# MDFahimAnjum/AliasFree-Diffusion-Models-PyTorch

Measured on AMD Instinct MI355X. Metric: train_step_images_per_sec, higher is better.
Workload: dtype f32; 1 GPU; CIFAR-10 32x32x3 synthetic, UNet variant=3 (Config D), batch 256/GPU, T=1000, AdamW lr 3e-4, random-init weights (seed 42); global_batch=256, parallelism=dp1, hip_graph=True, launch_mode=lanes

## Files before the change

### aliasfree-diffusion-models-pytorch_amd/csrc/conv.hip

```cpp
#include <cstdlib>
#include <algorithm>
#include "common.h"

namespace afd {

using f32x16 = __attribute__((ext_vector_type(16))) float;

static inline int gs_grid(long total, int block = 256) {
  long g = (total + block - 1) / block;
  return (int)(g < 1 ? 1 : (g > 65536 ? 65536 : g));
}

template <int KS>
__global__ void conv_direct_fwd(const float* __restrict__ x, const float* __restrict__ w, const float* __restrict__ bias,
                                const float* __restrict__ res, float* __restrict__ y,
                                int Cin, int Cout, int H, int W, int act, long total) {
  constexpr int T = KS * KS, R = KS / 2;
  for (long i = blockIdx.x * (long)blockDim.x + threadIdx.x; i < total; i += (long)gridDim.x * blockDim.x) {
    const int xx = i % W, yy = (i / W) % H;
    const long bc = i / ((long)W * H);
    const int co = bc % Cout; const long b = bc / Cout;
    float acc = bias ? bias[co] : 0.f;
    for (int ci = 0; ci < Cin; ++ci) {
      const float* xp = x + (b * Cin + ci) * (long)H * W;
// ... 695 lines not shown
  if (nb > 0) d[nd++] = afd_fold_desc{bp, db, (long)nb, (long)nb, (long)nb, 1L, slabs, accumulate};
  if (sink) {
    for (int i = 0; i < nd; ++i) sink->out[sink->n++] = d[i];
    return AFD_OK;
  }
  return fold_launch(d, nd, s);
}

bool pw_launch(const float* in, const float* w, const float* bias, const float* res, float* out, int B, int K, int N, int P,
               int act, bool dgrad, hipStream_t s);
void pw_set_mode(int m);
int wino_plan(int B, int K, int N, int H, int W);
int wino_conv(const float* x, const float* w, const float* bias, const float* res, float* y, float* U, int B, int K, int N, int H,
               int W, int act, bool dgrad, bool weights_ready, hipStream_t s);
void wino_set_mode(int m);
void wino_weights_launch(const float* w, float* Uf, float* Ud, int Cin, int Cout, int kinds, hipStream_t s);
bool bf3_ok(int B, int K, int N, int H, int W);
void bf3_set_mode(int m);
void direct_form_set(int m);
bool direct_form_is_bf3();
void h2_sk_set_mode(int m);
void h2_lds_set(int m);
void h2_skw_set(int m);
void wino_weights_batched_launch(const afd_wino_desc* descs, const int* wg_desc, int n_wg, hipStream_t s);
void wino_set_grid(int g);
int wgrad_wino_plan(int B, int Cin, int Cout, int H, int W, int* bn, int* bk, int* cps, int* nchunks);
int wgrad_bf3_plan(int B, int Cin, int Cout, int H, int W, int* tps, int* ntiles);
int wgrad_bf3(const float* x, const float* dy, float* part, int B, int Cin, int Cout, int H, int W, hipStream_t s);
void wgrad_bf3_set_mode(int m);
void wgrad_arith_set(int m);
void wgrad_plan_target_set(long wgs);
bool wgrad_arith_is_bf3();
int wgrad_h2(const float* x, const float* dy, float* part, int B, int Cin, int Cout, int H, int W, hipStream_t s);
int pw_wgrad_h2(const float* x, const float* dy, float* part, float* bias_part, int B, int Cin, int Cout, int L, hipStream_t s);
bool ends_fwd(const float* x, const float* w, const float* bias, const float* res, float* y, int B, int Cin, int Cout, int H, int W,
              int ksize, int act, hipStream_t s);
bool ends_dgrad(const float* dy, const float* w, float* dx, int B, int Cin, int Cout, int H, int W, int ksize, hipStream_t s);
void ends_set_mode(int m);
int wgrad_cin3_plan(int B, int Cin, int Cout, int H, int W);
int wgrad_cin3(const float* x, const float* dy, float* part, int B, int Cin, int Cout, int H, int W, hipStream_t s);
void pw_wgrad_bf3_set_mode(int m);
int pw_wgrad_bf3_plan(int B, int Cin, int Cout, int L, int* sps, int* nsteps, int* nr, int* nt);
int pw_wgrad_bf3(const float* x, const float* dy, float* part, float* bias_part, int B, int Cin, int Cout, int L, hipStream_t s);
int wgrad_wino(const float* x, const float* dy, float* part, int B, int Cin, int Cout, int H, int W, hipStream_t s);
void wgrad_wino_set_mode(int m);

static inline bool use_mfma(int K, int N, int H, int W, int PT) { return N >= 8 && tile_ok(H, W, PT); }

static int g_conv_path = 0;

template <int T, bool DGRAD>
static int launch_mfma(const float* x, const float* w, const float* bias, const float* res, float* y,
                       int B, int K, int N, int H, int W, int act, hipStream_t s) {
  constexpr int KC = (T == 9) ? 8 : 32;
  const long P = (long)B * H * W;
  if (P * K >= (1L << 31) || (long)K * N * T >= (1L << 31)) return -1;
  const unsigned ptiles = (unsigned)((P + 127) / 128);
  const long wgs64 = (long)ptiles * ((N + 63) / 64), wgs32 = (long)ptiles * ((N + 31) / 32);
  bool use32 = N <= 32 || (wgs64 < 256 && wgs32 >= 256);
  const bool want_sk = g_conv_path == 2 || (g_conv_path == 0 && wgs64 < 256 && wgs32 < 256);
  if (g_conv_path == 1) use32 = N <= 32;
  if (want_sk && K >= 32 && tile_ok(H, W, 64)) {
    const TileGeom g = make_geom(H, W, 64, T == 9 ? 1 : 0);
    if (g.XS <= 256) {
      const size_t lds_main = sizeof(float) * (32 * (32 * T + 1) + (size_t)32 * g.XS);
      const size_t lds_red = sizeof(float) * 4 * 2 * 16 * 64;
// ... 50 lines not shown

template <int T, int WNn, int WCn, int NPB>
static void launch_wgrad(const float* x, const float* dy, float* part, float* bias_part, int B, int Cin, int Cout, int H, int W,
                         const WgradPlan& p, const TileGeom& g, hipStream_t s) {
  const int nw = g_wgrad_nw ? g_wgrad_nw : ((p.cps >= 8 || (p.cps >= 4 && H * W >= 256)) ? 8 : 4);
  size_t lds = sizeof(float) * ((size_t)32 * WNn * 65 + (size_t)32 * WCn * (g.XS | 1)) + sizeof(int) * 64;
  const size_t red = sizeof(float) * nw * 16 * 64;
  if (WNn * WCn < nw && lds < red) lds = red;
  const dim3 grid((Cout + 32 * WNn - 1) / (32 * WNn), (Cin + 32 * WCn - 1) / (32 * WCn), p.splits);
  if (nw == 8)
    hipLaunchKernelGGL((conv_wgrad_mfma<T, WNn, WCn, NPB, 8>), grid, dim3(512), lds, s, x, dy, part, bias_part, B, Cin, Cout, H, W, p.cps, p.nchunks, g);
  else
    hipLaunchKernelGGL((conv_wgrad_mfma<T, WNn, WCn, NPB, 4>), grid, dim3(256), lds, s, x, dy, part, bias_part, B, Cin, Cout, H, W, p.cps, p.nchunks, g);
}

template <int T, int NPB>
static void launch_wgrad_roles(const float* x, const float* dy, float* part, float* bp, int B, int Cin, int Cout, int H, int W,
                               const WgradPlan& p, const TileGeom& g, hipStream_t s) {
  if (p.wnn == 2 && p.wcn == 2) launch_wgrad<T, 2, 2, NPB>(x, dy, part, bp, B, Cin, Cout, H, W, p, g, s);
  else if (p.wnn == 2) launch_wgrad<T, 2, 1, NPB>(x, dy, part, bp, B, Cin, Cout, H, W, p, g, s);
  else if (p.wcn == 2) launch_wgrad<T, 1, 2, NPB>(x, dy, part, bp, B, Cin, Cout, H, W, p, g, s);
  else launch_wgrad<T, 1, 1, NPB>(x, dy, part, bp, B, Cin, Cout, H, W, p, g, s);
}

}
using namespace afd;

extern "C" {

int afd_debug_conv_path(int mode) {
  if (mode >= 92 && mode <= 93) { ends_set_mode(mode - 92); return AFD_OK; }
  if (mode >= 88 && mode <= 89) { pw_wgrad_bf3_set_mode(mode - 88); return AFD_OK; }
  if (mode >= 84 && mode <= 86) { wgrad_bf3_set_mode(mode - 84); return AFD_OK; }
  if (mode >= 48 && mode <= 49) { wgrad_plan_target_set(mode == 48 ? 256 : 160); return AFD_OK; }
  if (mode >= 59 && mode <= 63) { h2_lds_set(mode == 59 ? 4 : (mode == 60 ? 1 : (mode == 61 ? 0 : mode - 60))); return AFD_OK; }
  if (mode == 73) { h2_sk_set_mode(2); return AFD_OK; }
  if (mode >= 71 && mode <= 72) { h2_skw_set(mode - 70); return AFD_OK; }
  if (mode == 74) h2_skw_set(0);
  if (mode >= 74 && mode <= 75) { h2_sk_set_mode(mode - 74); return AFD_OK; }
  if (mode >= 78 && mode <= 79) { wgrad_arith_set(mode - 78); return AFD_OK; }
  if (mode >= 76 && mode <= 77) { direct_form_set(mode - 76); return AFD_OK; }
  if (mode >= 80 && mode <= 82) { bf3_set_mode(mode - 80); return AFD_OK; }
  if (mode >= 8 && mode <= 10) { pw_set_mode(mode - 8); return AFD_OK; }
  if (mode >= 100000 && mode < 200000) { wino_set_grid(mode - 100000); return AFD_OK; }
  if (mode >= 96 && mode <= 98) { wgrad_wino_set_mode(mode - 96); return AFD_OK; }
  if (mode >= 64 && mode <= 70) { wino_set_mode(mode - 64); return AFD_OK; }
  if (mode >= 32 && mode <= 34) { g_wgrad_nw = mode == 32 ? 4 : (mode == 33 ? 8 : 0); return AFD_OK; }
  AFD_REQUIRE(mode >= 0 && mode <= 2, "afd_debug_conv_path: mode must be 0 (auto), 1 (big tile), 2 (split-K tile), 8..10 (1x1 streaming auto/off/forced), 32..34 (wgrad waves 4/8/auto), 64..69 (Winograd fwd/dgrad auto/off/forced shapes) or 96..98 (Winograd wgrad auto/off/forced)");
  g_conv_path = mode;
  return AFD_OK;
}

int afd_conv_fwd(const float* x, const float* w, const float* bias, const float* res, float* y,
                 int B, int Cin, int Cout, int H, int W, int ksize, int act, afd_stream_t st) {
  AFD_REQUIRE(x && w && y && B > 0 && Cin > 0 && Cout > 0 && H > 0 && W > 0, "afd_conv_fwd: bad argument");
  AFD_REQUIRE(ksize == 1 || ksize == 3, "afd_conv_fwd: ksize %d not in {1,3}", ksize);
  AFD_REQUIRE(act == 0 || act == 1, "afd_conv_fwd: act must be 0 or 1");
  hipStream_t s = as_stream(st);
  if (ends_fwd(x, w, bias, res, y, B, Cin, Cout, H, W, ksize, act, s)) return check_launch("afd_conv_fwd");
  if (ksize == 1 && pw_launch(x, w, bias, res, y, B, Cin, Cout, H * W, act, false, s)) return check_launch("afd_conv_fwd");
  int rc = -1;
  if (use_mfma(Cin, Cout, H, W, 128))
    rc = ksize == 3 ? launch_mfma<9, false>(x, w, bias, res, y, B, Cin, Cout, H, W, act, s)
                    : launch_mfma<1, false>(x, w, bias, res, y, B, Cin, Cout, H, W, act, s);
  if (rc != 0) {
    const long total = (long)B * Cout * H * W;
// ... 92 lines not shown
    const size_t ws = (size_t)wgrad_wino_plan(B, Cin, Cout, H, W, &bn, &bk, &cps, &nch);
    if (ws > slabs) slabs = ws;
    const size_t wb = (size_t)wgrad_bf3_plan(B, Cin, Cout, H, W, &cps, &nch);
    if (wb > slabs) slabs = wb;
    const size_t wc = (size_t)wgrad_cin3_plan(B, Cin, Cout, H, W);
    if (wc > slabs) slabs = wc;
  }
  const size_t need = slabs * ((size_t)Cout * Cin * ksize * ksize + Cout);
  const size_t direct = (size_t)B * Cout;
  return std::max(pw, sizeof(float) * (need > direct ? need : direct));
}

int afd_conv_wgrad_form(int B, int Cin, int Cout, int H, int W, int ksize) {
  if (B <= 0 || Cin <= 0 || Cout <= 0 || H <= 0 || W <= 0) return 0;
  int a, b, c, d;
  if (ksize == 1) return pw_wgrad_bf3_plan(B, Cin, Cout, H * W, &a, &b, &c, &d) ? (wgrad_arith_is_bf3() ? 2 : 4) : 0;
  if (ksize != 3) return 0;
  if (wgrad_bf3_plan(B, Cin, Cout, H, W, &a, &b)) return wgrad_arith_is_bf3() ? 2 : 4;
  if (wgrad_cin3_plan(B, Cin, Cout, H, W)) return 3;
  return wgrad_wino_plan(B, Cin, Cout, H, W, &a, &b, &c, &d) ? 1 : 0;
}

static int conv_wgrad_impl(const float* x, const float* dy, float* dw, float* dbias, int B, int Cin, int Cout, int H, int W,
                           int ksize, int accumulate, void* workspace, FoldSink* sink, hipStream_t s, const char* who) {
  AFD_REQUIRE(x && dy && dw && B > 0 && Cin > 0 && Cout > 0 && H > 0 && W > 0, "%s: bad argument", who);
  AFD_REQUIRE(ksize == 1 || ksize == 3, "%s: ksize %d not in {1,3}", who, ksize);
  const int T = ksize * ksize;
  const TileGeom g = make_geom(H, W, 64, ksize == 3 ? 1 : 0);
  int rc = AFD_OK;
  const bool vec = aligned16(x) && aligned16(dy);
  if (ksize == 3 && !dbias && workspace) {
    float* part = static_cast<float*>(workspace);
    int slabs = !vec ? 0 : (wgrad_arith_is_bf3() ? wgrad_bf3(x, dy, part, B, Cin, Cout, H, W, s) : wgrad_h2(x, dy, part, B, Cin, Cout, H, W, s));
    if (!slabs) slabs = wgrad_cin3(x, dy, part, B, Cin, Cout, H, W, s);
    if (!slabs && vec) slabs = wgrad_wino(x, dy, part, B, Cin, Cout, H, W, s);
    if (slabs) {
      const long n = (long)Cout * Cin * 9;
      rc = launch_wgrad_reduce(part, dw, n, slabs, nullptr, nullptr, 0, accumulate, 9, s, sink);
      return rc != AFD_OK ? rc : check_launch(who);
    }
  }
  if (ksize == 1 && workspace && vec) {
    int a, b, c, d;
    const int slabs = pw_wgrad_bf3_plan(B, Cin, Cout, H * W, &a, &b, &c, &d);
    if (slabs) {
      float* part = static_cast<float*>(workspace);
      const long n = (long)Cout * Cin;
      float* bp = dbias ? part + (size_t)slabs * n : nullptr;
      if (wgrad_arith_is_bf3()) pw_wgrad_bf3(x, dy, part, bp, B, Cin, Cout, H * W, s);
      else pw_wgrad_h2(x, dy, part, bp, B, Cin, Cout, H * W, s);
      rc = launch_wgrad_reduce(part, dw, n, slabs, bp, dbias, dbias ? Cout : 0, accumulate, 1, s, sink);
      return rc != AFD_OK ? rc : check_launch(who);
    }
  }
  if (tile_ok(H, W, 64) && g.XS <= 256 && (long)B * H * W * (Cin > Cout ? Cin : Cout) < (1L << 31)) {
    AFD_REQUIRE(workspace, "%s: workspace is NULL", who);
    const WgradPlan p = wgrad_plan(B, Cin, Cout, H, W, ksize);
    float* part = static_cast<float*>(workspace);
    const long n = (long)Cout * Cin * T;
    float* bp = dbias ? part + (size_t)p.slabs * n : nullptr;
    if (ksize == 1) launch_wgrad_roles<1, 2>(x, dy, part, bp, B, Cin, Cout, H, W, p, g, s);
    else if (p.npb == 4) launch_wgrad_roles<9, 4>(x, dy, part, bp, B, Cin, Cout, H, W, p, g, s);
    else if (p.npb == 5) launch_wgrad_roles<9, 5>(x, dy, part, bp, B, Cin, Cout, H, W, p, g, s);
    else launch_wgrad_roles<9, 8>(x, dy, part, bp, B, Cin, Cout, H, W, p, g, s);
    rc = launch_wgrad_reduce(part, dw, n, p.slabs, bp, dbias, dbias ? Cout : 0, accumulate, T, s, sink);
    return rc != AFD_OK ? rc : check_launch(who);
// ... 31 lines not shown
```

### aliasfree-diffusion-models-pytorch_amd/csrc/h2_wgrad.hip

```cpp
#include <algorithm>
#include <cstdint>
#include <cstdlib>
#include "common.h"
#include "h2_common.h"

namespace afd {

using f32x4 = __attribute__((ext_vector_type(4))) float;
using u32x4 = __attribute__((ext_vector_type(4))) uint32_t;

template <int S, int BN_, int BK_> struct HwGeo {
  static constexpr int TP = 128, G8 = S / 8;
  static constexpr int IPT = S * S >= TP ? 1 : TP / (S * S);
  static constexpr int R = S * S >= TP ? TP / S : S;
  static constexpr int TPI = S * S >= TP ? S * S / TP : 1;
  static constexpr int IG = (R + 2) * G8, NG = IPT * IG;
  static constexpr int BK = BK_, BN = BN_;
  static constexpr int NR = (BN / 16) * (BK / 32), NSG = 8 / NR;
  static constexpr int TASKS = (BK / 16) * NG * 16, NE = (TASKS + 511) / 512;
  static constexpr int PIECE = (BK / 16) * NG * 16;
};

__device__ __forceinline__ uint32_t h_pack(_Float16 lo, _Float16 hi) {
  return (uint32_t)__builtin_bit_cast(uint16_t, lo) | ((uint32_t)__builtin_bit_cast(uint16_t, hi) << 16);
}

template <int NR, int NSG>
__device__ __forceinline__ void hw_finish(f32x4 (&acc)[2][9], float unscale_x, float unscale_d, uint8_t* smem_raw, float* __restrict__ part,
                                          int split, int role, int sg, int lane, int n0w, int k0w, int N, int K) {
  const int l15 = lane & 15, kgl = lane >> 4;
#pragma unroll
  for (int ks = 0; ks < 2; ++ks)
#pragma unroll
    for (int t = 0; t < 9; ++t) acc[ks][t] = (acc[ks][t] * unscale_x) * unscale_d;
  if (NSG > 1) {
    float* red = reinterpret_cast<float*>(smem_raw);
#pragma unroll 1
    for (int g = 1; g < NSG; ++g) {
      __syncthreads();
      if (sg == g) {
#pragma unroll
        for (int ks = 0; ks < 2; ++ks)
#pragma unroll
          for (int t = 0; t < 9; ++t)
#pragma unroll
            for (int rg = 0; rg < 4; ++rg) red[(role * 72 + (ks * 9 + t) * 4 + rg) * 64 + lane] = acc[ks][t][rg];
      }
      __syncthreads();
      if (sg == 0) {
#pragma unroll
        for (int ks = 0; ks < 2; ++ks)
#pragma unroll
          for (int t = 0; t < 9; ++t)
#pragma unroll
// ... 112 lines not shown
  };

  float dv[10];
  const float* dyw = dy + (long)(n0 + 16 * ns + l15) * HW;
  auto d_fetch = [&](int tile, int step) {
    const int img0 = G::IPT > 1 ? tile * G::IPT : tile / G::TPI;
    const int row0 = G::IPT > 1 ? 0 : (tile % G::TPI) * G::R;
    const int pg = 4 * step + kgl;
    const int i = pg / (G::R * G8), rem = pg - i * (G::R * G8), r = rem / G8, c8 = rem - r * G8;
    const bool ok = img0 + i < B;
    const float* p = dyw + (long)(img0 + i) * N * HW + (row0 + r) * S + c8 * 8;
    const float4 a = ok ? reinterpret_cast<const float4*>(p)[0] : make_float4(0.f, 0.f, 0.f, 0.f);
    const float4 b = ok ? reinterpret_cast<const float4*>(p)[1] : make_float4(0.f, 0.f, 0.f, 0.f);
    dv[1] = a.x; dv[2] = a.y; dv[3] = a.z; dv[4] = a.w; dv[5] = b.x; dv[6] = b.y; dv[7] = b.z; dv[8] = b.w;
    dv[0] = (G8 > 1 && ok && c8 > 0) ? p[-1] : 0.f;
    dv[9] = (G8 > 1 && ok && c8 < G8 - 1) ? p[8] : 0.f;
  };

  f32x4 acc[2][9];
#pragma unroll
  for (int ks = 0; ks < 2; ++ks)
#pragma unroll
    for (int t = 0; t < 9; ++t) acc[ks][t] = f32x4{0.f, 0.f, 0.f, 0.f};

  const int brec0 = ((2 * kh) * NG) * 16 + l15;
  auto b_group = [&](int step) {
    const int pg = 4 * step + kgl;
    const int i = pg / (G::R * G8), rem = pg - i * (G::R * G8), r = rem / G8, c8 = rem - r * G8;
    return i * G::IG + (r + 1) * G8 + c8;
  };

  float sx = __uint_as_float(kH2ScaleCapBits), sd = sx;
  if (tbeg < tend) { x_fetch(tbeg); d_fetch(tbeg, sg); }
  for (int tile = tbeg; tile < tend; ++tile) {
    x_amax();
    __syncthreads();
    {
      float m = wmax[0];
#pragma unroll
      for (int q = 1; q < 8; ++q) m = fmaxf(m, wmax[q]);
      hw_rescale(acc, sx, m);
    }
    x_commit(sx);
    __syncthreads();
    if (tile + 1 < tend) x_fetch(tile + 1);
#pragma unroll 1
    for (int step = sg; step < 4; step += NSG) {
      {
        float m = 0.f;
#pragma unroll
        for (int j = 0; j < 10; ++j) m = fmaxf(m, fabsf(dv[j]));
        hw_rescale(acc, sd, wave_amax(m));
      }
      _Float16 pc[2][10];
#pragma unroll
      for (int j = 0; j < 10; ++j) h2_split(dv[j], sd, pc[0][j], pc[1][j]);
      h8 af[3][2];
#pragma unroll
      for (int p = 0; p < 2; ++p) {
        u32x4 e0, e1, e2;
#pragma unroll
        for (int q = 0; q < 4; ++q) {
          e0[q] = h_pack(pc[p][2 * q + 2], pc[p][2 * q + 3]);
          e1[q] = h_pack(pc[p][2 * q + 1], pc[p][2 * q + 2]);
          e2[q] = h_pack(pc[p][2 * q], pc[p][2 * q + 1]);
        }
        af[0][p] = __builtin_bit_cast(h8, e0); af[1][p] = __builtin_bit_cast(h8, e1); af[2][p] = __builtin_bit_cast(h8, e2);
      }
      if (step + NSG < 4) d_fetch(tile, step + NSG); else if (tile + 1 < tend) d_fetch(tile + 1, sg);

      hw_step(acc, af, Xs, PIECE, brec0 + b_group(step) * 16, NG * 16, -G8 * 16, 0, G8 * 16);
    }
  }

  hw_finish<G::NR, NSG>(acc, h2_inv_pow2(sx), h2_inv_pow2(sd), smem_raw, part, split, role, sg, lane, n0 + 16 * ns, k0 + 32 * kh, N, K);
}


template <int BN, int BK>
__global__ __launch_bounds__(512, 1) void wgrad_h2_s4(const float* __restrict__ x, const float* __restrict__ dy, float* __restrict__ part,
                                                       int B, int K, int N, int tiles_per_split, int ntiles) {
  constexpr int NR = (BN / 16) * (BK / 32), NSG = 8 / NR, NG = 40, PIECE = (BK / 16) * NG * 16, TASKS = 8 * BK;
  extern __shared__ __attribute__((aligned(16))) uint8_t smem_raw[];
  h8* Xs = reinterpret_cast<h8*>(smem_raw);
  float* wmax = reinterpret_cast<float*>(smem_raw + (size_t)2 * PIECE * 16);
  const int tid = threadIdx.x, lane = tid & 63, wv = tid >> 6, l15 = lane & 15, kgl = lane >> 4;
  const int role = wv % NR, sg = wv / NR;
  const int ns = role % (BN / 16), kh = role / (BN / 16);
  const int nkb = blockIdx.y, nbk = N / BN;
  const int n0 = (nkb % nbk) * BN, k0 = (nkb / nbk) * BK;
  const int split = blockIdx.x;
  const int tbeg = split * tiles_per_split, tend = min(ntiles, tbeg + tiles_per_split);

  const bool has_task = tid < TASKS;
  const int ti = tid / BK, tc = tid % BK;
  float xr[16];
  auto x_fetch = [&](int tile) {
    const int img = tile * 8 + ti;
    const bool ok = has_task && img < B;
    const float4* p = reinterpret_cast<const float4*>(x + ((long)(ok ? img : 0) * K + k0 + tc) * 16);
#pragma unroll
    for (int q = 0; q < 4; ++q) {
      const float4 v = ok ? p[q] : make_float4(0.f, 0.f, 0.f, 0.f);
      xr[4 * q] = v.x; xr[4 * q + 1] = v.y; xr[4 * q + 2] = v.z; xr[4 * q + 3] = v.w;
    }
  };
// ... 60 lines not shown
    x_commit(sx);
    __syncthreads();
    if (tile + 1 < tend) x_fetch(tile + 1);
#pragma unroll 1
    for (int step = sg; step < 4; step += NSG) {
      {
        float m = 0.f;
#pragma unroll
        for (int j = 0; j < 8; ++j) m = fmaxf(m, fabsf(dv[j]));
        hw_rescale(acc, sd, wave_amax(m));
      }
      _Float16 pc[2][8];
#pragma unroll
      for (int j = 0; j < 8; ++j) h2_split(dv[j], sd, pc[0][j], pc[1][j]);
      const _Float16 Z = (_Float16)0.f;
      h8 af[3][2];
#pragma unroll
      for (int p = 0; p < 2; ++p)
#pragma unroll
        for (int j = 0; j < 8; ++j) {
          af[1][p][j] = pc[p][j];
          af[0][p][j] = (j & 3) == 3 ? Z : pc[p][(j + 1) & 7];
          af[2][p][j] = (j & 3) == 0 ? Z : pc[p][(j + 7) & 7];
        }
      if (step + NSG < 4) d_fetch(tile, step + NSG); else if (tile + 1 < tend) d_fetch(tile + 1, sg);
      const int gb = brec0 + ((2 * step + (kgl >> 1)) * 5 + (kgl & 1)) * 16;
      hw_step(acc, af, Xs, PIECE, gb, NG * 16, 2 * 16, 0, 3 * 16);
    }
  }
  hw_finish<NR, NSG>(acc, h2_inv_pow2(sx), h2_inv_pow2(sd), smem_raw, part, split, role, sg, lane, n0 + 16 * ns, k0 + 32 * kh, N, K);
}


template <int NT>
__global__ __launch_bounds__(512, 1) void pw_wgrad_h2(const float* __restrict__ x, const float* __restrict__ dy, float* __restrict__ part,
                                                      float* __restrict__ bias_part, int B, int K, int N, int L, int steps_per_split,
                                                      int nsteps, int NR) {
  extern __shared__ __attribute__((aligned(16))) uint8_t smem_raw[];
  const int tid = threadIdx.x, lane = tid & 63, wv = tid >> 6, l15 = lane & 15, kgl = lane >> 4;
  const int WP = 8 / NR;
  const int role = blockIdx.y * NR + wv % NR, wp = wv / NR;
  const int ntn = N / (16 * NT);
  const int n0 = (role % ntn) * 16 * NT, k0 = (role / ntn) * 32;
  const int split = blockIdx.x;
  const int sbeg = split * steps_per_split, send = min(nsteps, sbeg + steps_per_split);

  f32x4 acc[NT][2];
  float bsum[NT];
#pragma unroll
  for (int i = 0; i < NT; ++i) { bsum[i] = 0.f; acc[i][0] = f32x4{0.f, 0.f, 0.f, 0.f}; acc[i][1] = acc[i][0]; }

  float4 ra[NT][2], rb[2][2];
  auto fetch = [&](int t) {
    const long P0 = 32L * t + 8 * kgl;
    const long b = P0 / L, p = P0 - b * L;
#pragma unroll
    for (int i = 0; i < NT; ++i) {
      const float4* q = reinterpret_cast<const float4*>(dy + (b * N + n0 + 16 * i + l15) * L + p);
      ra[i][0] = q[0]; ra[i][1] = q[1];
    }
#pragma unroll
    for (int j = 0; j < 2; ++j) {
      const float4* q = reinterpret_cast<const float4*>(x + (b * K + k0 + 16 * j + l15) * L + p);
      rb[j][0] = q[0]; rb[j][1] = q[1];
    }
  };
// ... 65 lines not shown
#pragma unroll
        for (int j = 0; j < 2; ++j)
#pragma unroll
          for (int rg = 0; rg < 4; ++rg) red[(rl * (NT * 9) + (i * 2 + j) * 4 + rg) * 64 + lane] = acc[i][j][rg];
        red[(rl * (NT * 9) + NT * 8 + i) * 64 + lane] = bsum[i];
      }
    }
    __syncthreads();
    if (wp == 0) {
#pragma unroll
      for (int i = 0; i < NT; ++i) {
#pragma unroll
        for (int j = 0; j < 2; ++j)
#pragma unroll
          for (int rg = 0; rg < 4; ++rg) acc[i][j][rg] += red[(rl * (NT * 9) + (i * 2 + j) * 4 + rg) * 64 + lane];
        bsum[i] += red[(rl * (NT * 9) + NT * 8 + i) * 64 + lane];
      }
    }
  }
  if (wp != 0) return;
  float* ps = part + (long)split * N * K;
#pragma unroll
  for (int i = 0; i < NT; ++i)
#pragma unroll
    for (int j = 0; j < 2; ++j)
#pragma unroll
      for (int rg = 0; rg < 4; ++rg) ps[(long)(n0 + 16 * i + 4 * kgl + rg) * K + k0 + 16 * j + l15] = acc[i][j][rg];
  if (bias_part && k0 == 0 && kgl == 0) {
#pragma unroll
    for (int i = 0; i < NT; ++i) bias_part[(long)split * N + n0 + 16 * i + l15] = bsum[i];
  }
}

int wgrad_bf3_plan(int B, int Cin, int Cout, int H, int W, int* tps, int* ntiles);
void wgrad_bf3_tile_for(int Cin, int Cout, long nt, int* bn, int* bk);

template <int S, int BN, int BK>
static void wgrad_h2_launch_t(const float* x, const float* dy, float* part, int B, int Cin, int Cout, int tps, int nt, int splits,
                              hipStream_t s) {
  using G = HwGeo<S, BN, BK>;
  const size_t lds = std::max((size_t)2 * G::PIECE * 16 + 32, G::NSG > 1 ? sizeof(float) * G::NR * 72 * 64 : (size_t)0);
  (void)lds_opt_in(&wgrad_h2<S, BN, BK>, lds);
  hipLaunchKernelGGL((wgrad_h2<S, BN, BK>), dim3((unsigned)splits, (unsigned)((Cout / BN) * (Cin / BK))), dim3(512), lds, s, x, dy,
                     part, B, Cin, Cout, tps, nt);
}

template <int BN, int BK>
static void wgrad_h2_s4_launch_t(const float* x, const float* dy, float* part, int B, int Cin, int Cout, int tps, int nt, int splits,
                                 hipStream_t s) {
  constexpr int NR = (BN / 16) * (BK / 32);
  const size_t lds = std::max((size_t)2 * (BK / 16) * 40 * 16 * 16 + 32, 8 / NR > 1 ? sizeof(float) * NR * 72 * 64 : (size_t)0);
  (void)lds_opt_in(&wgrad_h2_s4<BN, BK>, lds);
  hipLaunchKernelGGL((wgrad_h2_s4<BN, BK>), dim3((unsigned)splits, (unsigned)((Cout / BN) * (Cin / BK))), dim3(512), lds, s, x, dy, part, B,
                     Cin, Cout, tps, nt);
}

int wgrad_h2(const float* x, const float* dy, float* part, int B, int Cin, int Cout, int H, int W, hipStream_t s) {
  int tps, nt;
  const int splits = wgrad_bf3_plan(B, Cin, Cout, H, W, &tps, &nt);
  if (!splits) return 0;
  int bn_, bk_;
  wgrad_bf3_tile_for(Cin, Cout, nt, &bn_, &bk_);
  const bool n64 = bn_ == 64, k64 = bk_ == 64;
#define AFD_WGH(S_)                                                                                      \
  if (n64 && k64) wgrad_h2_launch_t<S_, 64, 64>(x, dy, part, B, Cin, Cout, tps, nt, splits, s);          \
  else if (n64) wgrad_h2_launch_t<S_, 64, 32>(x, dy, part, B, Cin, Cout, tps, nt, splits, s);            \
  else if (k64) wgrad_h2_launch_t<S_, 32, 64>(x, dy, part, B, Cin, Cout, tps, nt, splits, s);            \
  else wgrad_h2_launch_t<S_, 32, 32>(x, dy, part, B, Cin, Cout, tps, nt, splits, s)
  if (W == 32) { AFD_WGH(32); } else if (W == 16) { AFD_WGH(16); } else if (W == 8) { AFD_WGH(8); }
  else if (n64 && k64) wgrad_h2_s4_launch_t<64, 64>(x, dy, part, B, Cin, Cout, tps, nt, splits, s);
  else if (n64) wgrad_h2_s4_launch_t<64, 32>(x, dy, part, B, Cin, Cout, tps, nt, splits, s);
  else if (k64) wgrad_h2_s4_launch_t<32, 64>(x, dy, part, B, Cin, Cout, tps, nt, splits, s);
  else wgrad_h2_s4_launch_t<32, 32>(x, dy, part, B, Cin, Cout, tps, nt, splits, s);
#undef AFD_WGH
  return splits;
}


int pw_wgrad_bf3_plan(int B, int Cin, int Cout, int L, int* sps, int* nsteps, int* nr, int* nt);
int pw_wgrad_h2(const float* x, const float* dy, float* part, float* bias_part, int B, int Cin, int Cout, int L, hipStream_t s) {
  int sps, st, NR, NT;
  const int splits = pw_wgrad_bf3_plan(B, Cin, Cout, L, &sps, &st, &NR, &NT);
  if (!splits) return 0;
  const int roles = (Cout / (16 * NT)) * (Cin / 32);
  const size_t lds = 8 / NR > 1 ? sizeof(float) * NR * NT * 9 * 64 : 0;
  const dim3 grid((unsigned)splits, (unsigned)(roles / NR));
  if (NT == 3) hipLaunchKernelGGL(pw_wgrad_h2<3>, grid, dim3(512), lds, s, x, dy, part, bias_part, B, Cin, Cout, L, sps, st, NR);
  else hipLaunchKernelGGL(pw_wgrad_h2<2>, grid, dim3(512), lds, s, x, dy, part, bias_part, B, Cin, Cout, L, sps, st, NR);
  return splits;
}

}
```

Baseline: 40420 images/s.

## Add double-buffered pipelined h2 wgrad kernels with per-wave lazy dy rescaling

Adds new wgrad_h2p and wgrad_h2p_s4 kernels that double-buffer the x tile in LDS. Staging of the next tile (commit and prefetch) is interleaved between MFMA steps, staggered across early and late waves, so the second barrier per tile goes away. dy scaling now uses a per-wave ballot check before rescaling instead of a block-wide step, and a shape-based rule picks the pipelined form by default for some tile configs. The cost is doubled LDS for x staging, more register pressure, and extra accumulator rescale multiplies. It also adds optional timing stamps and error propagation from the LDS opt-in.

New measurement: 40430 images/s (median of 2 runs). About the same (+0.0%).

```diff
diff --git a/aliasfree-diffusion-models-pytorch_amd/csrc/conv.hip b/aliasfree-diffusion-models-pytorch_amd/csrc/conv.hip
--- a/aliasfree-diffusion-models-pytorch_amd/csrc/conv.hip
+++ b/aliasfree-diffusion-models-pytorch_amd/csrc/conv.hip
@@ -751,6 +751,7 @@
 void wgrad_plan_target_set(long wgs);
 bool wgrad_arith_is_bf3();
 int wgrad_h2(const float* x, const float* dy, float* part, int B, int Cin, int Cout, int H, int W, hipStream_t s);
+void wgrad_h2_form_set(int m);
 int pw_wgrad_h2(const float* x, const float* dy, float* part, float* bias_part, int B, int Cin, int Cout, int L, hipStream_t s);
 bool ends_fwd(const float* x, const float* w, const float* bias, const float* res, float* y, int B, int Cin, int Cout, int H, int W,
               int ksize, int act, hipStream_t s);
@@ -867,6 +868,7 @@
   if (mode >= 92 && mode <= 93) { ends_set_mode(mode - 92); return AFD_OK; }
   if (mode >= 88 && mode <= 89) { pw_wgrad_bf3_set_mode(mode - 88); return AFD_OK; }
   if (mode >= 84 && mode <= 86) { wgrad_bf3_set_mode(mode - 84); return AFD_OK; }
+  if (mode >= 52 && mode <= 55) { wgrad_h2_form_set(mode - 52); return AFD_OK; }
   if (mode >= 48 && mode <= 49) { wgrad_plan_target_set(mode == 48 ? 256 : 160); return AFD_OK; }
   if (mode >= 59 && mode <= 63) { h2_lds_set(mode == 59 ? 4 : (mode == 60 ? 1 : (mode == 61 ? 0 : mode - 60))); return AFD_OK; }
   if (mode == 73) { h2_sk_set_mode(2); return AFD_OK; }
@@ -1025,6 +1027,7 @@
   if (ksize == 3 && !dbias && workspace) {
     float* part = static_cast<float*>(workspace);
     int slabs = !vec ? 0 : (wgrad_arith_is_bf3() ? wgrad_bf3(x, dy, part, B, Cin, Cout, H, W, s) : wgrad_h2(x, dy, part, B, Cin, Cout, H, W, s));
+    if (slabs < 0) return -slabs;
     if (!slabs) slabs = wgrad_cin3(x, dy, part, B, Cin, Cout, H, W, s);
     if (!slabs && vec) slabs = wgrad_wino(x, dy, part, B, Cin, Cout, H, W, s);
     if (slabs) {
diff --git a/aliasfree-diffusion-models-pytorch_amd/csrc/h2_wgrad.hip b/aliasfree-diffusion-models-pytorch_amd/csrc/h2_wgrad.hip
--- a/aliasfree-diffusion-models-pytorch_amd/csrc/h2_wgrad.hip
+++ b/aliasfree-diffusion-models-pytorch_amd/csrc/h2_wgrad.hip
@@ -20,6 +20,29 @@
   static constexpr int TASKS = (BK / 16) * NG * 16, NE = (TASKS + 511) / 512;
   static constexpr int PIECE = (BK / 16) * NG * 16;
 };
+
+#ifndef AFD_WGH_STAMP
+#define AFD_WGH_STAMP 0
+#endif
+#if AFD_WGH_STAMP
+constexpr int kWghStampWgs = 1024;
+__device__ unsigned long long g_wgh_stamps[kWghStampWgs * 8 * 4];
+struct WghClock {
+  unsigned long long t, acc[4];
+  __device__ __forceinline__ WghClock() : t(__builtin_amdgcn_s_memtime()), acc{0, 0, 0, 0} {}
+  __device__ __forceinline__ void lap(int k) { const unsigned long long n = __builtin_amdgcn_s_memtime(); acc[k] += n - t; t = n; }
+  __device__ __forceinline__ void dump(int wv, int lane) const {
+    const unsigned wg = blockIdx.y * gridDim.x + blockIdx.x;
+    if (lane == 0 && wg < (unsigned)kWghStampWgs)
+      for (int k = 0; k < 4; ++k) g_wgh_stamps[(wg * 8 + wv) * 4 + k] = acc[k];
+  }
+};
+#else
+struct WghClock {
+  __device__ __forceinline__ void lap(int) {}
+  __device__ __forceinline__ void dump(int, int) const {}
+};
+#endif
 
 __device__ __forceinline__ uint32_t h_pack(_Float16 lo, _Float16 hi) {
   return (uint32_t)__builtin_bit_cast(uint16_t, lo) | ((uint32_t)__builtin_bit_cast(uint16_t, hi) << 16);
@@ -198,9 +221,12 @@
 
   float sx = __uint_as_float(kH2ScaleCapBits), sd = sx;
   if (tbeg < tend) { x_fetch(tbeg); d_fetch(tbeg, sg); }
+  WghClock clk;
   for (int tile = tbeg; tile < tend; ++tile) {
     x_amax();
+    clk.lap(0);
     __syncthreads();
+    clk.lap(1);
     {
       float m = wmax[0];
 #pragma unroll
@@ -208,8 +234,11 @@
       hw_rescale(acc, sx, m);
     }
     x_commit(sx);
+    clk.lap(0);
     __syncthreads();
+    clk.lap(1);
     if (tile + 1 < tend) x_fetch(tile + 1);
+    clk.lap(0);
 #pragma unroll 1
     for (int step = sg; step < 4; step += NSG) {
       {
@@ -234,10 +263,13 @@
         af[0][p] = __builtin_bit_cast(h8, e0); af[1][p] = __builtin_bit_cast(h8, e1); af[2][p] = __builtin_bit_cast(h8, e2);
       }
       if (step + NSG < 4) d_fetch(tile, step + NSG); else if (tile + 1 < tend) d_fetch(tile + 1, sg);
+      clk.lap(2);
 
       hw_step(acc, af, Xs, PIECE, brec0 + b_group(step) * 16, NG * 16, -G8 * 16, 0, G8 * 16);
-    }
-  }
+      clk.lap(3);
+    }
+  }
+  clk.dump(wv, lane);
 
   hw_finish<G::NR, NSG>(acc, h2_inv_pow2(sx), h2_inv_pow2(sd), smem_raw, part, split, role, sg, lane, n0 + 16 * ns, k0 + 32 * kh, N, K);
 }
@@ -364,6 +396,410 @@
 }
 
 
+using h2v = __attribute__((ext_vector_type(2))) _Float16;
+using f2v = __attribute__((ext_vector_type(2))) float;
+
+__device__ __forceinline__ void h2_split_pk(float x0, float x1, float s, uint32_t& p0, uint32_t& p1) {
+  const f2v v = f2v{x0, x1} * s;
+  const h2v a = __builtin_convertvector(v, h2v);
+  const h2v b = __builtin_convertvector(v - __builtin_convertvector(a, f2v), h2v);
+  p0 = __builtin_bit_cast(uint32_t, a); p1 = __builtin_bit_cast(uint32_t, b);
+}
+__device__ __forceinline__ void h2_split8_pk(const float (&x)[8], float s, h8& p0, h8& p1) {
+  uint32_t a[4], b[4];
+#pragma unroll
+  for (int q = 0; q < 4; ++q) h2_split_pk(x[2 * q], x[2 * q + 1], s, a[q], b[q]);
+  p0 = __builtin_bit_cast(h8, (u32x4{a[0], a[1], a[2], a[3]})); p1 = __builtin_bit_cast(h8, (u32x4{b[0], b[1], b[2], b[3]}));
+}
+__device__ __forceinline__ float amax3(float m, float a, float b) { return fmaxf(fmaxf(m, fabsf(a)), fabsf(b)); }
+
+__device__ __forceinline__ void hw_fit(f32x4 (&acc)[2][9], float& s, float& lim, float m) {
+  if (__builtin_amdgcn_ballot_w64(!(m < lim)) != 0ull) {
+    hw_rescale(acc, s, wave_amax(m));
+    lim = 32768.f * h2_inv_pow2(s);
+  }
+}
+
+template <int S, int BN, int BK, int NBUF>
+__global__ __launch_bounds__(512, 1) void wgrad_h2p(const float* __restrict__ x, const float* __restrict__ dy, float* __restrict__ part,
+                                                     int B, int K, int N, int tiles_per_split, int ntiles) {
+  using G = HwGeo<S, BN, BK>;
+  constexpr int HW = S * S, G8 = G::G8, NG = G::NG, NE = G::NE, PIECE = G::PIECE, NSG = G::NSG, SPW = 4 / NSG;
+  extern __shared__ __attribute__((aligned(16))) uint8_t smem_raw[];
+  h8* Xs = reinterpret_cast<h8*>(smem_raw);
+  float* wmax = reinterpret_cast<float*>(smem_raw + (size_t)NBUF * 2 * PIECE * 16);
+  const int tid = threadIdx.x, lane = tid & 63, l15 = lane & 15, kgl = lane >> 4;
+  const int wv = __builtin_amdgcn_readfirstlane(tid >> 6);
+  const int role = wv % G::NR, sg = wv / G::NR;
+  const int ns = role % (BN / 16), kh = role / (BN / 16);
+  const int nkb = blockIdx.y, nbk = N / G::BN;
+  const int n0 = (nkb % nbk) * G::BN, k0 = (nkb / nbk) * G::BK;
+  const int split = blockIdx.x;
+  const int tbeg = split * tiles_per_split, tend = min(ntiles, tbeg + tiles_per_split);
+
+  int s_off[NE], s_rr[NE];
+#pragma unroll
+  for (int e = 0; e < NE; ++e) {
+    const int t = tid + 512 * e;
+    s_rr[e] = -1; s_off[e] = 0;
+    if (t < G::TASKS) {
+      const int c16 = t & 15, g = (t >> 4) % NG, ksub = t / (16 * NG);
+      const int i = g / G::IG, rem = g - i * G::IG, rr = rem / G8, c8 = rem - rr * G8;
+      s_rr[e] = rr | (i << 8);
+      s_off[e] = (i * K + ksub * 16 + c16) * HW + (rr - 1) * S + c8 * 8;
+    }
+  }
+  float xr[NE][8];
+  auto x_fetch = [&](int tile) {
+    const int img0 = G::IPT > 1 ? tile * G::IPT : tile / G::TPI;
+    const int row0 = G::IPT > 1 ? 0 : (tile % G::TPI) * G::R;
+    const float* xb = x + ((long)img0 * K + k0) * HW + row0 * S;
+#pragma unroll
+    for (int e = 0; e < NE; ++e) {
+      const int rr = s_rr[e] & 255, i = s_rr[e] >> 8, yy = row0 + rr - 1;
+      const bool ok = s_rr[e] >= 0 && yy >= 0 && yy < S && img0 + i < B;
+      const float4* p = reinterpret_cast<const float4*>(xb + (ok ? s_off[e] : 0));
+      const float4 a = ok ? p[0] : make_float4(0.f, 0.f, 0.f, 0.f), b = ok ? p[1] : make_float4(0.f, 0.f, 0.f, 0.f);
+      xr[e][0] = a.x; xr[e][1] = a.y; xr[e][2] = a.z; xr[e][3] = a.w; xr[e][4] = b.x; xr[e][5] = b.y; xr[e][6] = b.z; xr[e][7] = b.w;
+    }
+  };
+  auto x_amax = [&](int buf) {
+    float m = 0.f;
+#pragma unroll
+    for (int e = 0; e < NE; ++e)
+#pragma unroll
+      for (int j = 0; j < 8; j += 2) m = amax3(m, xr[e][j], xr[e][j + 1]);
+    m = wave_amax(m);
+    if (lane == 0) wmax[buf * 8 + wv] = m;
+  };
+  auto x_max8 = [&](int buf) {
+    float m = wmax[buf * 8];
+#pragma unroll
+    for (int q = 1; q < 8; ++q) m = fmaxf(m, wmax[buf * 8 + q]);
+    return m;
+  };
+  auto x_commit = [&](int buf, float s) {
+    h8* Xb = Xs + buf * (2 * PIECE);
+#pragma unroll
+    for (int e = 0; e < NE; ++e) {
+      if (s_rr[e] < 0) continue;
+      h8 p0, p1;
+      h2_split8_pk(xr[e], s, p0, p1);
+      const int t = tid + 512 * e;
+      Xb[t] = p0; Xb[PIECE + t] = p1;
+    }
+  };
+
+  const int c8 = kgl & (G8 - 1);
+  const bool has_l = G8 > 1 && c8 > 0, has_r = G8 > 1 && c8 < G8 - 1;
+  const uint32_t dl = (uint32_t)((n0 + 16 * ns + l15) * HW + kgl * 8);
+  const uint32_t dl_l = has_l ? dl - 1 : dl, dl_r = has_r ? dl + 8 : dl;
+  float dv[SPW][10];
+  auto d_fetch = [&](int tile, int j, float (&d)[10]) {
+    const int step = sg + j * NSG;
+    const int img = G::IPT > 1 ? tile * G::IPT + (step >> 1) : tile / G::TPI;
+    const int off = G::IPT > 1 ? (step & 1) * 32 : (tile % G::TPI) * G::R * S + step * 32;
+    if (G::IPT > 1 && img >= B) {
+#pragma unroll
+      for (int q = 0; q < 10; ++q) d[q] = 0.f;
+      return;
+    }
+    const float* p = dy + ((long)img * N * HW + off);
+    const float4 a = *reinterpret_cast<const float4*>(p + dl), b = *reinterpret_cast<const float4*>(p + dl + 4);
+    d[1] = a.x; d[2] = a.y; d[3] = a.z; d[4] = a.w; d[5] = b.x; d[6] = b.y; d[7] = b.z; d[8] = b.w;
+    if (G8 > 1) {
+      const float l = p[dl_l], r = p[dl_r];
+      d[0] = has_l ? l : 0.f; d[9] = has_r ? r : 0.f;
+    } else {
+      d[0] = 0.f; d[9] = 0.f;
+    }
+  };
+
+  f32x4 acc[2][9];
+#pragma unroll
+  for (int ks = 0; ks < 2; ++ks)
+#pragma unroll
+    for (int t = 0; t < 9; ++t) acc[ks][t] = f32x4{0.f, 0.f, 0.f, 0.f};
+
+  const int brec0 = ((2 * kh) * NG + (S == 32 ? 4 : (S == 16 ? 2 : 1)) + kgl) * 16 + l15;
+  auto b_step = [&](int step) { return (S >= 16 ? 4 * step : (step >> 1) * G::IG + 4 * (step & 1)) * 16; };
+
+  float sx = __uint_as_float(kH2ScaleCapBits), sd = sx, limd = 0.f;
+  WghClock clk;
+  auto step_do = [&](int tile, int j, const h8* Xb) {
+    float (&d)[10] = dv[j];
+    {
+      float m = 0.f;
+#pragma unroll
+      for (int q = 0; q < 10; q += 2) m = amax3(m, d[q], d[q + 1]);
+      hw_fit(acc, sd, limd, m);
+    }
+    uint32_t e[2][5];
+#pragma unroll
+    for (int k = 0; k < 5; ++k) h2_split_pk(d[2 * k], d[2 * k + 1], sd, e[0][k], e[1][k]);
+    h8 af[3][2];
+#pragma unroll
+    for (int p = 0; p < 2; ++p) {
+      u32x4 e0, e1, e2;
+#pragma unroll
+      for (int q = 0; q < 4; ++q) {
+        e0[q] = e[p][q + 1];
+        e1[q] = __builtin_amdgcn_alignbit(e[p][q + 1], e[p][q], 16);
+        e2[q] = e[p][q];
+      }
+      af[0][p] = __builtin_bit_cast(h8, e0); af[1][p] = __builtin_bit_cast(h8, e1); af[2][p] = __builtin_bit_cast(h8, e2);
+    }
+    d_fetch(min(tile + 1, tend - 1), j, d);
+    clk.lap(2);
+    hw_step(acc, af, Xb, PIECE, brec0 + b_step(sg + j * NSG), NG * 16, -G8 * 16, 0, G8 * 16);
+    clk.lap(3);
+  };
+
+  if (tbeg < tend) {
+    x_fetch(tbeg);
+#pragma unroll
+    for (int j = 0; j < SPW; ++j) d_fetch(tbeg, j, dv[j]);
+  }
+  if (NBUF == 1) {
+#pragma unroll 1
+    for (int tile = tbeg; tile < tend; ++tile) {
+      x_amax(0);
+      clk.lap(0);
+      __syncthreads();
+      clk.lap(1);
+      hw_rescale(acc, sx, x_max8(0));
+      x_commit(0, sx);
+      clk.lap(0);
+      __syncthreads();
+      clk.lap(1);
+      if (tile + 1 < tend) x_fetch(tile + 1);
+      clk.lap(0);
+#pragma unroll
+      for (int j = 0; j < SPW; ++j) step_do(tile, j, Xs);
+    }
+  } else {
+    const bool late = wv >= 4;
+    int buf = 0;
+    if (tbeg < tend) {
+      x_amax(0);
+      __syncthreads();
+      hw_rescale(acc, sx, x_max8(0));
+      x_commit(0, sx);
+      if (tbeg + 1 < tend) x_fetch(tbeg + 1);
+    }
+#pragma unroll 1
+    for (int tile = tbeg; tile < tend; ++tile, buf ^= 1) {
+      const bool more = tile + 1 < tend;
+      if (more) x_amax(buf ^ 1);
+      clk.lap(0);
+      __syncthreads();
+      clk.lap(1);
+      float sxn = sx;
+      if (more) sxn = fminf(sx, h2_scale_for(x_max8(buf ^ 1)));
+      auto stage = [&]() {
+        if (more) {
+          x_commit(buf ^ 1, sxn);
+          if (tile + 2 < tend) x_fetch(tile + 2);
+        }
+        clk.lap(0);
+      };
+      const h8* Xb = Xs + buf * (2 * PIECE);
+#pragma unroll
+      for (int j = 0; j < SPW; ++j) {
+        if (j == 0 && !late) stage();
+        if (SPW > 1 && j == SPW / 2 && late) stage();
+        step_do(tile, j, Xb);
+      }
+      if (SPW == 1 && late) stage();
+      if (sxn != sx) {
+        const float f = sxn * h2_inv_pow2(sx);
+#pragma unroll
+        for (int ks = 0; ks < 2; ++ks)
+#pragma unroll
+          for (int t = 0; t < 9; ++t) acc[ks][t] *= f;
+        sx = sxn;
+      }
+    }
+  }
+
+  clk.dump(wv, lane);
+  hw_finish<G::NR, NSG>(acc, h2_inv_pow2(sx), h2_inv_pow2(sd), smem_raw, part, split, role, sg, lane, n0 + 16 * ns, k0 + 32 * kh, N, K);
+}
+
+template <int BN, int BK, int NBUF>
+__global__ __launch_bounds__(512, 1) void wgrad_h2p_s4(const float* __restrict__ x, const float* __restrict__ dy, float* __restrict__ part,
+                                                        int B, int K, int N, int tiles_per_split, int ntiles) {
+  constexpr int NR = (BN / 16) * (BK / 32), NSG = 8 / NR, SPW = 4 / NSG, NG = 40, PIECE = (BK / 16) * NG * 16, TASKS = 8 * BK;
+  extern __shared__ __attribute__((aligned(16))) uint8_t smem_raw[];
+  h8* Xs = reinterpret_cast<h8*>(smem_raw);
+  float* wmax = reinterpret_cast<float*>(smem_raw + (size_t)NBUF * 2 * PIECE * 16);
+  const int tid = threadIdx.x, lane = tid & 63, l15 = lane & 15, kgl = lane >> 4;
+  const int wv = __builtin_amdgcn_readfirstlane(tid >> 6);
+  const int role = wv % NR, sg = wv / NR;
+  const int ns = role % (BN / 16), kh = role / (BN / 16);
+  const int nkb = blockIdx.y, nbk = N / BN;
+  const int n0 = (nkb % nbk) * BN, k0 = (nkb / nbk) * BK;
+  const int split = blockIdx.x;
+  const int tbeg = split * tiles_per_split, tend = min(ntiles, tbeg + tiles_per_split);
+
+  const bool has_task = tid < TASKS;
+  const int ti = tid / BK, tc = tid % BK;
+  float xr[16];
+  auto x_fetch = [&](int tile) {
+    const int img = tile * 8 + ti;
+    const bool ok = has_task && img < B;
+    const float4* p = reinterpret_cast<const float4*>(x + ((long)(ok ? img : 0) * K + k0 + tc) * 16);
+#pragma unroll
+    for (int q = 0; q < 4; ++q) {
+      const float4 v = ok ? p[q] : make_float4(0.f, 0.f, 0.f, 0.f);
+      xr[4 * q] = v.x; xr[4 * q + 1] = v.y; xr[4 * q + 2] = v.z; xr[4 * q + 3] = v.w;
+    }
+  };
+  auto x_amax = [&](int buf) {
+    float m = 0.f;
+#pragma unroll
+    for (int j = 0; j < 16; j += 2) m = amax3(m, xr[j], xr[j + 1]);
+    m = wave_amax(m);
+    if (lane == 0) wmax[buf * 8 + wv] = m;
+  };
+  auto x_max8 = [&](int buf) {
+    float m = wmax[buf * 8];
+#pragma unroll
+    for (int q = 1; q < 8; ++q) m = fmaxf(m, wmax[buf * 8 + q]);
+    return m;
+  };
+  auto x_commit = [&](int buf, float s) {
+    if (!has_task) return;
+    uint32_t pk[2][8];
+#pragma unroll
+    for (int k = 0; k < 8; ++k) h2_split_pk(xr[2 * k], xr[2 * k + 1], s, pk[0][k], pk[1][k]);
+    const int rec = (((tc >> 4) * 8 + ti) * 5) * 16 + (tc & 15);
+#pragma unroll
+    for (int p = 0; p < 2; ++p) {
+      const uint32_t* q = pk[p];
+      h8* d = Xs + buf * (2 * PIECE) + p * PIECE + rec;
+      d[0] = __builtin_bit_cast(h8, (u32x4{q[0], q[1], q[2], q[3]}));
+      d[16] = __builtin_bit_cast(h8, (u32x4{q[4], q[5], q[6], q[7]}));
+      d[32] = __builtin_bit_cast(h8, (u32x4{0u, 0u, q[0], q[1]}));
+      d[48] = __builtin_bit_cast(h8, (u32x4{q[2], q[3], q[4], q[5]}));
+      d[64] = __builtin_bit_cast(h8, (u32x4{q[6], q[7], 0u, 0u}));
+    }
+  };
+
+  const uint32_t dl = (uint32_t)(((kgl >> 1) * N + n0 + 16 * ns + l15) * 16 + (kgl & 1) * 8);
+  float dv[SPW][8];
+  auto d_fetch = [&](int tile, int j, float (&d)[8]) {
+    const int img = tile * 8 + 2 * (sg + j * NSG);
+    float4 a, b;
+    if (img + 1 < B) {
+      const float* p = dy + (long)img * N * 16;
+      a = *reinterpret_cast<const float4*>(p + dl); b = *reinterpret_cast<const float4*>(p + dl + 4);
+    } else {
+      const bool ok = img + (kgl >> 1) < B;
+      const float* p = dy + (long)(img < B ? img : 0) * N * 16;
+      const uint32_t o = ok ? dl : 0u;
+      a = *reinterpret_cast<const float4*>(p + o); b = *reinterpret_cast<const float4*>(p + o + 4);
+      if (!ok) { a = make_float4(0.f, 0.f, 0.f, 0.f); b = a; }
+    }
+    d[0] = a.x; d[1] = a.y; d[2] = a.z; d[3] = a.w; d[4] = b.x; d[5] = b.y; d[6] = b.z; d[7] = b.w;
+  };
+
+  f32x4 acc[2][9];
+#pragma unroll
+  for (int ks = 0; ks < 2; ++ks)
+#pragma unroll
+    for (int t = 0; t < 9; ++t) acc[ks][t] = f32x4{0.f, 0.f, 0.f, 0.f};
+  const int brec0 = ((2 * kh) * NG + (kgl >> 1) * 5 + (kgl & 1)) * 16 + l15;
+
+  float sx = __uint_as_float(kH2ScaleCapBits), sd = sx, limd = 0.f;
+  auto step_do = [&](int tile, int j, const h8* Xb) {
+    float (&d)[8] = dv[j];
+    {
+      float m = 0.f;
+#pragma unroll
+      for (int q = 0; q < 8; q += 2) m = amax3(m, d[q], d[q + 1]);
+      hw_fit(acc, sd, limd, m);
+    }
+    uint32_t e[2][4];
+#pragma unroll
+    for (int k = 0; k < 4; ++k) h2_split_pk(d[2 * k], d[2 * k + 1], sd, e[0][k], e[1][k]);
+    h8 af[3][2];
+#pragma unroll
+    for (int p = 0; p < 2; ++p) {
+      const uint32_t m01 = __builtin_amdgcn_alignbit(e[p][1], e[p][0], 16), m23 = __builtin_amdgcn_alignbit(e[p][3], e[p][2], 16);
+      af[1][p] = __builtin_bit_cast(h8, (u32x4{e[p][0], e[p][1], e[p][2], e[p][3]}));
+      af[0][p] = __builtin_bit_cast(h8, (u32x4{m01, e[p][1] >> 16, m23, e[p][3] >> 16}));
+      af[2][p] = __builtin_bit_cast(h8, (u32x4{e[p][0] << 16, m01, e[p][2] << 16, m23}));
+    }
+    d_fetch(min(tile + 1, tend - 1), j, d);
+    hw_step(acc, af, Xb, PIECE, brec0 + (sg + j * NSG) * 10 * 16, NG * 16, 2 * 16, 0, 3 * 16);
+  };
+
+  if (!has_task) {
+#pragma unroll
+    for (int j = 0; j < 16; ++j) xr[j] = 0.f;
+  }
+  if (tbeg < tend) {
+    x_fetch(tbeg);
+#pragma unroll
+    for (int j = 0; j < SPW; ++j) d_fetch(tbeg, j, dv[j]);
+  }
+  if (NBUF == 1) {
+#pragma unroll 1
+    for (int tile = tbeg; tile < tend; ++tile) {
+      x_amax(0);
+      __syncthreads();
+      hw_rescale(acc, sx, x_max8(0));
+      x_commit(0, sx);
+      __syncthreads();
+      if (tile + 1 < tend) x_fetch(tile + 1);
+#pragma unroll
+      for (int j = 0; j < SPW; ++j) step_do(tile, j, Xs);
+    }
+  } else {
+    const bool late = wv >= 4;
+    int buf = 0;
+    if (tbeg < tend) {
+      x_amax(0);
+      __syncthreads();
+      hw_rescale(acc, sx, x_max8(0));
+      x_commit(0, sx);
+      if (tbeg + 1 < tend) x_fetch(tbeg + 1);
+    }
+#pragma unroll 1
+    for (int tile = tbeg; tile < tend; ++tile, buf ^= 1) {
+      const bool more = tile + 1 < tend;
+      if (more) x_amax(buf ^ 1);
+      __syncthreads();
+      float sxn = sx;
+      if (more) sxn = fminf(sx, h2_scale_for(x_max8(buf ^ 1)));
+      auto stage = [&]() {
+        if (more) {
+          x_commit(buf ^ 1, sxn);
+          if (tile + 2 < tend) x_fetch(tile + 2);
+        }
+      };
+      const h8* Xb = Xs + buf * (2 * PIECE);
+#pragma unroll
+      for (int j = 0; j < SPW; ++j) {
+        if (j == 0 && !late) stage();
+        if (SPW > 1 && j == SPW / 2 && late) stage();
+        step_do(tile, j, Xb);
+      }
+      if (SPW == 1 && late) stage();
+      if (sxn != sx) {
+        const float f = sxn * h2_inv_pow2(sx);
+#pragma unroll
+        for (int ks = 0; ks < 2; ++ks)
+#pragma unroll
+          for (int t = 0; t < 9; ++t) acc[ks][t] *= f;
+        sx = sxn;
+      }
+    }
+  }
+  hw_finish<NR, NSG>(acc, h2_inv_pow2(sx), h2_inv_pow2(sd), smem_raw, part, split, role, sg, lane, n0 + 16 * ns, k0 + 32 * kh, N, K);
+}
+
 template <int NT>
 __global__ __launch_bounds__(512, 1) void pw_wgrad_h2(const float* __restrict__ x, const float* __restrict__ dy, float* __restrict__ part,
                                                       float* __restrict__ bias_part, int B, int K, int N, int L, int steps_per_split,
@@ -495,27 +931,72 @@
   }
 }
 
+#if AFD_WGH_STAMP
+}
+extern "C" int afd_debug_wgh_stamps(unsigned long long* out, int n, int clear) {
+  using namespace afd;
+  const size_t bytes = sizeof(unsigned long long) * (size_t)std::min(n, kWghStampWgs * 8 * 4);
+  if (hipDeviceSynchronize() != hipSuccess) return AFD_ELAUNCH;
+  if (out && hipMemcpyFromSymbol(out, HIP_SYMBOL(g_wgh_stamps), bytes) != hipSuccess) return AFD_ELAUNCH;
+  if (clear) {
+    void* p = nullptr;
+    if (hipGetSymbolAddress(&p, HIP_SYMBOL(g_wgh_stamps)) != hipSuccess || hipMemset(p, 0, sizeof(g_wgh_stamps)) != hipSuccess) return AFD_ELAUNCH;
+  }
+  return AFD_OK;
+}
+namespace afd {
+#endif
+
 int wgrad_bf3_plan(int B, int Cin, int Cout, int H, int W, int* tps, int* ntiles);
 void wgrad_bf3_tile_for(int Cin, int Cout, long nt, int* bn, int* bk);
 
+static int wgrad_h2_rule(int S, int bn, int bk) {
+  if (S == 4) return bn == 32 && bk == 32 ? 2 : 0;
+  if (bn == 64 && bk == 64) return 2;
+  if (S == 32 && bn == 32 && bk == 64) return 2;
+  return 0;
+}
+static int g_wgh_form = -1;
+void wgrad_h2_form_set(int m) { g_wgh_form = m - 1; }
+static int wgrad_h2_form(int S, int bn, int bk) {
+  static const int env_form = [] { const char* e = getenv("AFD_WGH_FORM"); return e ? atoi(e) : -1; }();
+  int f = g_wgh_form >= 0 ? g_wgh_form : env_form;
+  if (f < 0 || f > 2) f = wgrad_h2_rule(S, bn, bk);
+  return (f == 2 && S == 4 && bk == 64) ? 1 : f;
+}
+
+template <class Kern>
+static int wgrad_h2_go(Kern kern, size_t lds, const float* x, const float* dy, float* part, int B, int Cin, int Cout, int BN, int BK,
+                       int tps, int nt, int splits, hipStream_t s) {
+  if (int rc = lds_opt_in(kern, lds)) return rc;
+  hipLaunchKernelGGL(kern, dim3((unsigned)splits, (unsigned)((Cout / BN) * (Cin / BK))), dim3(512), lds, s, x, dy, part, B, Cin, Cout, tps, nt);
+  return AFD_OK;
+}
+
 template <int S, int BN, int BK>
-static void wgrad_h2_launch_t(const float* x, const float* dy, float* part, int B, int Cin, int Cout, int tps, int nt, int splits,
-                              hipStream_t s) {
+static int wgrad_h2_launch_t(const float* x, const float* dy, float* part, int B, int Cin, int Cout, int tps, int nt, int splits,
+                             hipStream_t s) {
   using G = HwGeo<S, BN, BK>;
-  const size_t lds = std::max((size_t)2 * G::PIECE * 16 + 32, G::NSG > 1 ? sizeof(float) * G::NR * 72 * 64 : (size_t)0);
-  (void)lds_opt_in(&wgrad_h2<S, BN, BK>, lds);
-  hipLaunchKernelGGL((wgrad_h2<S, BN, BK>), dim3((unsigned)splits, (unsigned)((Cout / BN) * (Cin / BK))), dim3(512), lds, s, x, dy,
-                     part, B, Cin, Cout, tps, nt);
+  const size_t red = G::NSG > 1 ? sizeof(float) * G::NR * 72 * 64 : (size_t)0;
+  const int form = wgrad_h2_form(S, BN, BK);
+  const size_t lds = std::max((size_t)(form == 2 ? 2 : 1) * (2 * G::PIECE * 16 + 32), red);
+  if (form == 2) return wgrad_h2_go(&wgrad_h2p<S, BN, BK, 2>, lds, x, dy, part, B, Cin, Cout, BN, BK, tps, nt, splits, s);
+  if (form == 1) return wgrad_h2_go(&wgrad_h2p<S, BN, BK, 1>, lds, x, dy, part, B, Cin, Cout, BN, BK, tps, nt, splits, s);
+  return wgrad_h2_go(&wgrad_h2<S, BN, BK>, lds, x, dy, part, B, Cin, Cout, BN, BK, tps, nt, splits, s);
 }
 
 template <int BN, int BK>
-static void wgrad_h2_s4_launch_t(const float* x, const float* dy, float* part, int B, int Cin, int Cout, int tps, int nt, int splits,
-                                 hipStream_t s) {
+static int wgrad_h2_s4_launch_t(const float* x, const float* dy, float* part, int B, int Cin, int Cout, int tps, int nt, int splits,
+                                hipStream_t s) {
   constexpr int NR = (BN / 16) * (BK / 32);
-  const size_t lds = std::max((size_t)2 * (BK / 16) * 40 * 16 * 16 + 32, 8 / NR > 1 ? sizeof(float) * NR * 72 * 64 : (size_t)0);
-  (void)lds_opt_in(&wgrad_h2_s4<BN, BK>, lds);
-  hipLaunchKernelGGL((wgrad_h2_s4<BN, BK>), dim3((unsigned)splits, (unsigned)((Cout / BN) * (Cin / BK))), dim3(512), lds, s, x, dy, part, B,
-                     Cin, Cout, tps, nt);
+  const size_t red = 8 / NR > 1 ? sizeof(float) * NR * 72 * 64 : (size_t)0;
+  const int form = wgrad_h2_form(4, BN, BK);
+  const size_t lds = std::max((size_t)(form == 2 ? 2 : 1) * (2 * (BK / 16) * 40 * 16 * 16 + 32), red);
+  if constexpr (BK == 32) {
+    if (form == 2) return wgrad_h2_go(&wgrad_h2p_s4<BN, BK, 2>, lds, x, dy, part, B, Cin, Cout, BN, BK, tps, nt, splits, s);
+  }
+  if (form >= 1) return wgrad_h2_go(&wgrad_h2p_s4<BN, BK, 1>, lds, x, dy, part, B, Cin, Cout, BN, BK, tps, nt, splits, s);
+  return wgrad_h2_go(&wgrad_h2_s4<BN, BK>, lds, x, dy, part, B, Cin, Cout, BN, BK, tps, nt, splits, s);
 }
 
 int wgrad_h2(const float* x, const float* dy, float* part, int B, int Cin, int Cout, int H, int W, hipStream_t s) {
@@ -525,18 +1006,19 @@
   int bn_, bk_;
   wgrad_bf3_tile_for(Cin, Cout, nt, &bn_, &bk_);
   const bool n64 = bn_ == 64, k64 = bk_ == 64;
-#define AFD_WGH(S_)                                                                                      \
-  if (n64 && k64) wgrad_h2_launch_t<S_, 64, 64>(x, dy, part, B, Cin, Cout, tps, nt, splits, s);          \
-  else if (n64) wgrad_h2_launch_t<S_, 64, 32>(x, dy, part, B, Cin, Cout, tps, nt, splits, s);            \
-  else if (k64) wgrad_h2_launch_t<S_, 32, 64>(x, dy, part, B, Cin, Cout, tps, nt, splits, s);            \
-  else wgrad_h2_launch_t<S_, 32, 32>(x, dy, part, B, Cin, Cout, tps, nt, splits, s)
+  int rc;
+#define AFD_WGH(S_)                                                                                           \
+  if (n64 && k64) rc = wgrad_h2_launch_t<S_, 64, 64>(x, dy, part, B, Cin, Cout, tps, nt, splits, s);          \
+  else if (n64) rc = wgrad_h2_launch_t<S_, 64, 32>(x, dy, part, B, Cin, Cout, tps, nt, splits, s);            \
+  else if (k64) rc = wgrad_h2_launch_t<S_, 32, 64>(x, dy, part, B, Cin, Cout, tps, nt, splits, s);            \
+  else rc = wgrad_h2_launch_t<S_, 32, 32>(x, dy, part, B, Cin, Cout, tps, nt, splits, s)
   if (W == 32) { AFD_WGH(32); } else if (W == 16) { AFD_WGH(16); } else if (W == 8) { AFD_WGH(8); }
-  else if (n64 && k64) wgrad_h2_s4_launch_t<64, 64>(x, dy, part, B, Cin, Cout, tps, nt, splits, s);
-  else if (n64) wgrad_h2_s4_launch_t<64, 32>(x, dy, part, B, Cin, Cout, tps, nt, splits, s);
-  else if (k64) wgrad_h2_s4_launch_t<32, 64>(x, dy, part, B, Cin, Cout, tps, nt, splits, s);
-  else wgrad_h2_s4_launch_t<32, 32>(x, dy, part, B, Cin, Cout, tps, nt, splits, s);
+  else if (n64 && k64) rc = wgrad_h2_s4_launch_t<64, 64>(x, dy, part, B, Cin, Cout, tps, nt, splits, s);
+  else if (n64) rc = wgrad_h2_s4_launch_t<64, 32>(x, dy, part, B, Cin, Cout, tps, nt, splits, s);
+  else if (k64) rc = wgrad_h2_s4_launch_t<32, 64>(x, dy, part, B, Cin, Cout, tps, nt, splits, s);
+  else rc = wgrad_h2_s4_launch_t<32, 32>(x, dy, part, B, Cin, Cout, tps, nt, splits, s);
 #undef AFD_WGH
-  return splits;
+  return rc != AFD_OK ? -rc : splits;
 }
 
 
```
